# jiaowoguanren0615/Segmentation_Factory

Hardware: AMD Instinct MI355X
Metric: images/sec/GPU fwd+bwd SegFormer-B0 512x512 bf16; mIoU parity vs CPU ref (higher is better)
Workload: dtype bf16; 1 GPU; SegFormer-B0 (MiT-B0 + 768-wide SegFormerHead as the reference builds it), 150 classes, 512x512, full train step (zero_grad+fwd+CE/Dice+bwd+AGC/AdamW); per_gpu_batch=256, global_batch=256, parallelism=dp1, fp8=False, inputs=resident in HBM in the captured step's input buffers (zero-copy feed), launch=hipGraph(zero_grad+fwd+loss+bwd+grad gather) + RCCL all-reduce + fused AGC/AdamW

## Files before the change

### include/segfac.h

```cpp
#ifndef SEGFAC_H
#define SEGFAC_H
#include <stdint.h>

#ifdef __cplusplus
extern "C" {
#endif

#define SEGF_F32 0
#define SEGF_BF16 1
#define SEGF_ERR_SHAPE (-1)
#define SEGF_ERR_DTYPE (-2)
#define SEGF_ERR_WORKSPACE (-3)

const char* segf_version(void);

int segf_cast(const void* src, int src_dt, void* dst, int dst_dt, int64_t n, void* stream);
int segf_cast2d(const void* src, int src_dt, int64_t ld_src, void* dst, int dst_dt, int64_t ld_dst, int64_t rows, int64_t cols,
                void* stream);
int segf_permute021(const void* in, int in_dt, void* out, int out_dt, int64_t A, int64_t Bd, int64_t Cd,
                    int64_t ld_out, void* stream);
typedef struct SegfPrepItem {
    const void* src; void* dst;
    int64_t rows, cols, ld_src, ld_dst, pb, pc;
    int32_t op, src_dt, dst_dt, reserved;
// ... 119 lines not shown
                         float* ws, const void* x1, int64_t ldx1, int C1, float* dG, float* dwcls, void* stream);

int64_t segf_grn_ws(int B, int64_t rows_per_sample, int C, int bwd);
int segf_grn_fwd(int dt, int B, int64_t rows_per_sample, int C, const void* x, const float* gamma, const float* beta, void* y,
                 float* a_scratch, float* sumsq_out, float* ws, int pre_gelu, void* stream);
int segf_grn_bwd(int dt, int B, int64_t rows_per_sample, int C, const void* x, const void* dy, const float* gamma,
                 const float* sumsq_saved, void* dx, float* dgamma, float* dbeta, float* ws, int pre_gelu, void* stream);

int segf_attention_fwd(int dt, int B, int heads, int N, int Nkv, int hd, const void* q, int64_t ldq,
                       const void* k, int64_t ldk, const void* v, int64_t ldv, float scale,
                       void* o, int64_t ldo, float* lse, void* stream);
int64_t segf_attention_bwd_ws(int B, int heads, int N, int Nkv, int hd);
int segf_attention_bwd(int dt, int B, int heads, int N, int Nkv, int hd, const void* q, int64_t ldq,
                       const void* k, int64_t ldk, const void* v, int64_t ldv, float scale,
                       const void* o, int64_t ldo, const void* d_o, int64_t lddo, const float* lse,
                       void* dq, int64_t lddq, void* dk, int64_t lddk, void* dv, int64_t lddv,
                       float* ws, void* stream);

int segf_dwconv3x3_gelu_fwd(int dt, int B, int H, int W, int C, const void* x, const float* w ,
                            const float* bias, int apply_gelu, void* y, void* stream);
int64_t segf_dwconv3x3_bwd_ws(int B, int H, int W, int C);
int segf_dwconv3x3_bwd_blocks(int dt, int B, int H, int W, int C);
int segf_dwconv3x3_gelu_bwd(int dt, int B, int H, int W, int C, const void* x, const float* w, const float* bias,
                            int apply_gelu, const void* dy, void* du, void* dx, float* dw, float* db,
                            float* ws, void* stream);

int segf_dwconv7x7_fwd(int dt, int B, int H, int W, int C, const void* x, const float* wt, const float* bias, void* y,
                       void* stream);
int64_t segf_dwconv7x7_bwd_ws(int B, int H, int W, int C);
int segf_dwconv7x7_bwd(int dt, int B, int H, int W, int C, const void* x, const float* wt, const void* dy, void* dx,
                       float* dw, float* db, float* ws, void* stream);

int segf_conv3x3_fwd_splitk(int mode, int B, int H, int W, int Cin, int Cout);
int segf_conv3x3_pick_splitk(int Cin, int Cout, int64_t P);
int segf_conv3x3(int mode, int B, int H, int W, int Cin, int Cout, const void* x, int64_t ldx, const void* w, int64_t ldw,
                 void* y, int y_dt, int64_t ldy, const float* bias, int split_k, float* ws, void* stream);

int segf_gelu(int dt, int mode, const void* u, const void* dy, void* y, int64_t n, void* stream);
int segf_rowdot(const float* a, int64_t lda, const float* b, int64_t ldb, const float* extra_a, const float* extra_b,
                float* out, int64_t rows, int64_t cols, void* stream);
int segf_adaptive_avgpool(int dt, int bwd, int B, int H, int W, int C, int S, const void* in, void* out, void* stream);

int segf_im2col(int dt, int in_nchw_f32, int B, int H, int W, int Cin, int kh, int kw, int stride, int pad,
                int Ho, int Wo, const void* x, void* col, int64_t ldcol, void* stream);
int segf_col2im(int dt, int B, int H, int W, int Cin, int kh, int kw, int stride, int pad,
                int Ho, int Wo, const void* dcol, int64_t ldcol, void* dx, void* stream);

int segf_bilinear_fwd(int dt, int B, int h, int w, int C, const void* in, int64_t ldi,
                      int H, int W, void* out, int64_t ldo, int align_corners, void* stream);
int segf_bilinear_bwd(int dt, int B, int h, int w, int C, void* din, int64_t ldi,
                      int H, int W, const void* dout, int64_t ldo, int align_corners, void* stream);
int segf_bilinear_bwd_248(int dt, int B, int H, int W, int C, const void* dout, int64_t ldo, void* d2, void* d4, void* d8,
                          void* stream);
int segf_upsample_add(int dt, int B, int H, int W, int C, const void* base, int64_t ldb, int nsrc,
                      const void* src0, int h0, int w0, int64_t ld0, const void* src1, int h1, int w1, int64_t ld1,
                      const void* src2, int h2, int w2, int64_t ld2, void* out, int64_t ldo, int align_corners, void* stream);
int64_t segf_upsample_add_stats_ws(int B, int H, int W, int C);
int segf_upsample_add_stats(int dt, int B, int H, int W, int C, const void* base, int64_t ldb, int nsrc,
                            const void* src0, int h0, int w0, int64_t ld0, const void* src1, int h1, int w1, int64_t ld1,
                            const void* src2, int h2, int w2, int64_t ld2, void* out, int64_t ldo, int align_corners,
                            float* sums, float* ws, void* stream);
int segf_fuse_map_248_supported(int dt, int B, int H, int W, int C, int C1);
int64_t segf_fuse_map_248_ws(int B, int H, int W, int C);
int segf_fuse_map_248(int B, int H, int W, int C, int C1, const void* x1, int64_t ldx1, const void* g1, int64_t ldg,
                      const void* t2, int64_t ld2, const void* t3, int64_t ld3, const void* t4, int64_t ld4,
                      void* out, int64_t ldo, float* sums, float* ws, void* stream);
int segf_bn_stats_from_sums(const float* sums, int64_t rows, int C, float* mean, float* rstd, float* running_mean,
                            float* running_var, float momentum, float eps, void* stream);
int segf_nearest_up(int dt, int bwd, int B, int h, int w, int C, int H, int W, const void* in, const void* base, void* out,
                    void* stream);
int segf_bilinear_to_nchw_f32(int dt, int B, int h, int w, int C, const void* in, int64_t ldi,
                              int H, int W, float* out, void* stream);

int64_t segf_ce_dice_stats_floats(int B, int C);
int64_t segf_ce_dice_lse_floats(int dt, int B, int C, int h, int w, int H, int W, const void* logits, int64_t ldl);
int segf_ce_dice_fwd(int dt, int B, int C, int h, int w, int H, int W, const void* logits, int64_t ldl,
                     const int64_t* target, int64_t ignore_index, const float* class_weight, int dice,
                     float* stats, float* loss, float* pix_lse, void* stream);
int64_t segf_ce_dice_bwd_ws(int dt, int B, int C, int h, int w, int H, int W);
int segf_ce_dice_bwd(int dt, int B, int C, int h, int w, int H, int W, const void* logits, int64_t ldl,
                     const int64_t* target, int64_t ignore_index, const float* class_weight, int dice,
                     const float* stats, const float* grad_out, void* dlogits, int64_t ldd, float* ws,
                     const float* pix_lse, void* stream);

int segf_debug_wave_reduce16(const float* in, float* out, void* stream);

int segf_argmax_confmat(int dt, int B, int C, int h, int w, int H, int W, const void* logits, int64_t ldl,
                        const int64_t* target, int64_t ignore_label, int64_t* mat, int64_t* hist,
                        int32_t* flag, int64_t* pred_out , void* stream);

int segf_argmax_rows(int dt, int64_t rows, int C, const void* x, int64_t ld, int64_t* out, void* stream);

int segf_confmat_pairs(const int64_t* gt, const int64_t* pred, int64_t n, int C, int64_t ignore_label,
                       int64_t* mat, int64_t* hist, int32_t* flag, void* stream);

int segf_agc_adamw(float* param, const float* grad, float* exp_avg, float* exp_avg_sq,
                   const int64_t* unit_offset, const int32_t* unit_len, const uint8_t* unit_flags, int32_t* unit_step,
                   int nunits, float lr, float beta1, float beta2, float eps, float weight_decay, int step,
                   float clip_factor, float agc_eps, void* stream);

int64_t segf_clip_grad_ws(void);
int segf_clip_grad(float* grad, int64_t n, int mode, float value, float* ws, void* stream);

typedef struct {
    const uint8_t* img;
    const uint8_t* lbl;
// ... 28 lines not shown
```

### segmentation_factory_amd/csrc/fuse_map.hip

```cpp
#include <stdlib.h>
#include "colreduce.h"

typedef __attribute__((ext_vector_type(8))) __bf16 bf16x8;
typedef __attribute__((ext_vector_type(4))) float f32x4;
typedef __attribute__((ext_vector_type(4))) short s16x4;
typedef __attribute__((ext_vector_type(8))) short s16x8;
typedef uint32_t u32x4 __attribute__((ext_vector_type(4)));

#define FM_SLICE 128
#define FM_SROW 272
#define FM_NSRC 61
#ifndef FM_OCC
#define FM_OCC 2
#endif

struct FuseMapArgs {
    const bf16_t* x1; int64_t ldx1;
    const bf16_t* g1; int64_t ldg;
    const bf16_t *src0, *src1, *src2; int64_t ld0, ld1, ld2;
    bf16_t* out; int64_t ldo;
    float* partial;
    int B, H, W, C;
    int tiles_x, tiles_per_img; int64_t ntiles;
    FastDivU32 div_tx, div_tpi;
// ... 353 lines not shown
            SEGF_LOADS_ISSUED();
        }
        if (tx <= 1 || tx == w8 - 1) build_weights(tx);
#pragma unroll
        for (int ct = 0; ct < 2; ++ct) {
            const int cb = 16 * (2 * wave + ct);
            f32x4 acc0 = {0.f, 0.f, 0.f, 0.f}, acc1 = {0.f, 0.f, 0.f, 0.f};
#pragma unroll
            for (int s = 0; s < 8; ++s) {
                const unsigned char* tile = win + (s >> 1) * 16384;
                const int gp = g ^ phase, q = mi >> 2, pp = mi & 3;
                const int u = (cb >> 2) + pp, chunk = u >> 1, half = u & 1;
                const int kr0 = 32 * (s & 1) + 8 * gp + q, kr1 = kr0 + 4;
                const s16x4 lo = __builtin_amdgcn_ds_read_tr16_b64_v4i16(
                    (__attribute__((address_space(3))) s16x4*)(tile + kr0 * 256 + ((chunk ^ fm_swz(kr0)) << 4) + half * 8));
                const s16x4 hi = __builtin_amdgcn_ds_read_tr16_b64_v4i16(
                    (__attribute__((address_space(3))) s16x4*)(tile + kr1 * 256 + ((chunk ^ fm_swz(kr1)) << 4) + half * 8));
                const bf16x8 fa = __builtin_bit_cast(bf16x8, __builtin_shufflevector(lo, hi, 0, 1, 2, 3, 4, 5, 6, 7));
                if (s >= 1 && s <= 6) acc0 = __builtin_amdgcn_mfma_f32_16x16x32_bf16(fa, wb0[s - 1], acc0, 0, 0, 0);
                acc1 = __builtin_amdgcn_mfma_f32_16x16x32_bf16(fa, wb1[s], acc1, 0, 0, 0);
            }
            *reinterpret_cast<uint2*>(ost[0] + mi * FM_SROW + (cb + 4 * g) * 2) = make_uint2(pack2bf(acc0[0], acc0[1]), pack2bf(acc0[2], acc0[3]));
            *reinterpret_cast<uint2*>(ost[1] + mi * FM_SROW + (cb + 4 * g) * 2) = make_uint2(pack2bf(acc1[0], acc1[1]), pack2bf(acc1[2], acc1[3]));
        }
        __syncthreads();
        store_half(phase, sreg);
        {
            const int src = threadIdx.x >> 4;
            const uint4 o = *reinterpret_cast<const uint4*>(ost[0] + src * FM_SROW + 16 * ck);
            *reinterpret_cast<uint4*>(a.d2 + (((int64_t)b * h2 + 4 * ty + (src >> 2)) * w2 + 4 * tx + (src & 3)) * a.C + c0 + 8 * ck) = o;
            if (threadIdx.x < 80) {
                const uint4 o1 = *reinterpret_cast<const uint4*>(ost[1] + src * FM_SROW + 16 * ck);
                bf16_t* dst = src < 4 ? a.d4 + (((int64_t)b * h4 + 2 * ty + (src >> 1)) * w4 + 2 * tx + (src & 1)) * a.C
                                      : a.d8 + (((int64_t)b * h8 + ty) * w8 + tx) * a.C;
                *reinterpret_cast<uint4*>(dst + c0 + 8 * ck) = o1;
            }
        }
        __syncthreads();
    }
}

int fuse_map_bwd_supported(int dt, int B, int H, int W, int C) {
    return dt == SEGF_BF16 && B > 0 && H % 8 == 0 && W % 8 == 0 && H >= 8 && W >= 8 && C % FM_SLICE == 0 &&
           (int64_t)H * W < (1ll << 30) && !POL(no_bwd248_mfma);
}
int fuse_map_bwd_launch(int B, int H, int W, int C, const void* dy, int64_t ldo, void* d2, void* d4, void* d8, hipStream_t st) {
    FuseMapBwdArgs a{(const bf16_t*)dy, ldo, (bf16_t*)d2, (bf16_t*)d4, (bf16_t*)d8, B, H, W, C, C / FM_SLICE};
    const int64_t wgs = (int64_t)B * (H / 8) * a.nslice;
    if (wgs <= 0 || wgs >= (1ll << 31)) return SEGF_ERR_SHAPE;
    hipLaunchKernelGGL(fuse_map_bwd_kernel, dim3((unsigned)wgs), dim3(256), 0, st, a);
    SEGF_CHECK_LAUNCH();
    return 0;
}
```

### segmentation_factory_amd/csrc/policy.h

```cpp
#pragma once

#define SEGF_POLICY_TABLE(X)                                                                                                             \
                                                                                                   \
    X(gemm_no_big, "SEGFAC_GEMM_NO_BIG", 0, "never take the 256 x 256-tile kernel (gemm_bf16_big_kernel): everything on the 128-tile one") \
    X(gemm_no_skinny, "SEGFAC_GEMM_NO_SKINNY", 0, "no streaming products for K, N <= 128 (gemm_skinny_kernel and its relatives)")        \
    X(gemm_no_skinny_rows, "SEGFAC_GEMM_NO_SKINNY_ROWS", 0, "the [tokens x 32] -> 768 projection on gemm_skinny_kernel instead of the whole-row form") \
    X(gemm_no_skinny_k, "SEGFAC_GEMM_NO_SKINNY_K", 0, "no K-split streaming product for 32- / 64-wide outputs (gemm_skinny_k_kernel)")  \
    X(gemm_no_dw_skinny, "SEGFAC_GEMM_NO_DW_SKINNY", 0, "small-output weight gradients on the tiled split-K kernel instead of gemm_dw_skinny_kernel") \
    X(gemm_no_narrow, "SEGFAC_GEMM_NO_NARROW", 0, "256-tile kernel: full 128 x 64 wave tiles also for outputs <= 160 wide (bit-identical results)") \
    X(gemm_no_deep, "SEGFAC_GEMM_NO_DEEP", 0, "256-tile forward: one K step of operand loads in flight instead of two")                  \
    X(gemm_no_deep128, "SEGFAC_GEMM_NO_DEEP128", 0, "128-tile kernel: one K step in flight instead of two")                              \
    X(gemm_no_fastload, "SEGFAC_GEMM_NO_FASTLOAD", 0, "guarded tile loads everywhere (no workgroup-uniform guard-free full-K-step loads)") \
    X(gemm_no_tr, "SEGFAC_GEMM_NO_TR", 0, "debugging: reduction-major fragments by scalar LDS reads instead of ds_read_b64_tr_b16; disables every kernel built on the transposed read") \
    X(gemm_no_pro, "SEGFAC_GEMM_NO_PRO", 0, "segf_gemm_pro_supported answers 0: BatchNorm + ReLU + Dropout2d are applied by their own pass") \
    X(gemm_no_fused_db, "SEGFAC_GEMM_NO_FUSED_DB", 0, "bias gradient as its own column-sum launch instead of riding on the weight-gradient product") \
    X(no_grouped_dw, "SEGFAC_NO_GROUPED_DW", 0, "segf_gemm_dw_db_grouped runs its members one by one")                                   \
    X(dw_no_xcd_slabs, "SEGFAC_DW_NO_XCD_SLABS", 0, "split-K weight gradients (128-tile kernel) in hardware workgroup order instead of one K slab per XCD")                \
    X(dw_no_shared_split, "SEGFAC_DW_NO_SHARED_SPLIT", 0, "grouped weight gradients keep their per-layer slice counts (also read by the host layer)") \
    X(no_wide_reduce, "SEGFAC_NO_WIDE_REDUCE", 0, "split-K partials of large outputs summed by the 16 x 16 form instead of whole rows")   \
    X(no_reduce4, "SEGFAC_NO_REDUCE4", 0, "split-K reduce: one output per thread instead of four (bitwise the same sums)")               \
    X(gemm_f32_no_mfma, "SEGFAC_GEMM_F32_NO_MFMA", 0, "fp32 storage (exact-parity mode, evaluate): products on the vector FMA kernel instead of the f32 matrix instruction") \
    X(gemm8_linear, "SEGFAC_GEMM8_LINEAR", 1, "0: plain nn.Linear products never take the eight-phase kernel (the 256 / 128 tile kernels as in r04)") \
    X(gemm8_linear_min_tiles, "SEGFAC_GEMM8_LINEAR_MIN_TILES", 128, "fewest 256 x 256 tiles for which a K >= 2048 nn.Linear product takes the eight-phase kernel (192 for shorter K)") \
    X(gemm8_linear_min_fill, "SEGFAC_GEMM8_LINEAR_MIN_FILL", 60, "smallest share (percent) of the launched 256 x 256 tiles that must be output for an nn.Linear product with ragged last tiles to take the eight-phase kernel") \
    X(gemm8_linear_min_k, "SEGFAC_GEMM8_LINEAR_MIN_K", 256, "shortest reduction for which an nn.Linear product takes the eight-phase kernel (its 12-load prologue and drain against K / 64 tiles)") \
    X(gemm8_dw, "SEGFAC_GEMM8_DW", 1, "0: nn.Linear weight gradients never take the eight-phase kernel below 65536 tokens (the grouped 128-tile kernel as in r04)") \
    X(gemm8_dw_min_gflop, "SEGFAC_GEMM8_DW_MIN_GFLOP", 100, "smallest nn.Linear weight gradient (GFLOP; both feature counts multiples of 256, >= 256 FLOP per operand byte) that takes the eight-phase kernel + a column-sum pass instead of the grouped 128-tile kernel") \
    X(gemm8_linear_min_gflop, "SEGFAC_GEMM8_LINEAR_MIN_GFLOP", 36, "smallest nn.Linear product (GFLOP, K >= 512; 100 for shorter K) that takes the eight-phase kernel") \
                                 \
    X(no_gemm8, "SEGFAC_NO_GEMM8", 0, "no eight-phase kernel at all (gemm8_kernel): the two-phase 256-tile kernel everywhere")           \
    X(no_gemm8t, "SEGFAC_NO_GEMM8T", 0, "no eight-phase kernel for weight gradients (reduction-major operands)")                         \
    X(conv_no_fwd_split, "SEGFAC_CONV_NO_FWD_SPLIT", 0, "3 x 3 forward / data gradient with few output tiles: no split over the (channel block, tap) walk") \
    X(g8_stagger, "SEGFAC_G8_STAGGER", -1, "eight-phase kernel: 1 = wave groups one barrier apart, 0 = lockstep, -1 = staggered for bf16 and the per-device choice (segf_gemm8_option) for fp8") \
    X(no_fp8, "SEGFAC_NO_FP8", 0, "segf_gemm_fp8_supported answers 0 (block-scaled 128-tile fp8 GEMM)")                                  \
    X(no_fp8_conv, "SEGFAC_NO_FP8_CONV", 0, "segf_conv3x3_fp8*_supported answer 0")                                                      \
    X(no_fp8_wgrad, "SEGFAC_NO_FP8_WGRAD", 0, "fp8 3 x 3 convolutions keep a bf16 weight gradient")                                      \
    X(no_fp8_linear, "SEGFAC_NO_FP8_LINEAR", 0, "segf_linear_fp8_supported answers 0")                                                   \
                                                                            \
    X(attn_no_mfma, "SEGFAC_ATTN_NO_MFMA", 0, "attention on the VALU reference kernels (attention.hip) also in bf16")                    \
    X(attn_f32_no_mfma, "SEGFAC_ATTN_F32_NO_MFMA", 0, "fp32 attention forward on the vector kernel (one query per lane) instead of the f32 matrix instruction") \
    X(attn64_prescale, "SEGFAC_ATTN64_PRESCALE", 0, "head dim 64, >= 128 keys: scale log2(e) rides on the Q fragments (bf16(q c), one more rounding per q element) and -max / -lse are the score accumulators' initial values, instead of one multiply-add per score: forward + query-side backward, +8 % / +2 % per kernel, attention error x 1.2 - 2.3") \
    X(attn64_dkv_rows, "SEGFAC_ATTN64_DKV_ROWS", 128, "head dim 64, >= 128 keys, key-side backward: query rows per staged Q / dO tile and barrier (128, 64 or 32: the same arithmetic, bit for bit)") \
    X(attn_no_fused_bwd, "SEGFAC_ATTN_NO_FUSED_BWD", 0, "head dim 32, <= 256 keys: query-side + key-side backward kernels instead of the one-kernel backward") \
                                                                                \
    X(dw_no_walk, "SEGFAC_DW_NO_WALK", 0, "depthwise 3 x 3: the round-1 strip kernels instead of the vertical-walk kernels")             \
    X(dw_walk_rows, "SEGFAC_DW_WALK_ROWS", 0, "depthwise 3 x 3 walk: rows per segment (0 = chosen from the map size)")                   \
    X(dw_no_small, "SEGFAC_DW_NO_SMALL", 0, "depthwise 3 x 3 backward of small maps: three passes instead of the one-launch LDS form")   \
    X(dw_small_always, "SEGFAC_DW_SMALL_ALWAYS", 0, "... the one-launch form beyond one round of workgroups as well")                    \
                                                           \
    X(no_fuse_map, "SEGFAC_NO_FUSE_MAP", 0, "folded SegFormerHead map: streaming product + VALU upsample-add instead of fuse_map_kernel") \
    X(no_bwd248_mfma, "SEGFAC_NO_BWD248_MFMA", 0, "transposed 1/2-1/4-1/8 resizes on the VALU kernel instead of fuse_map_bwd_kernel")    \
    X(upadd_generic, "SEGFAC_UPADD_GENERIC", 0, "upsample-add: the generic per-source kernels also for the 2-4-8 pyramid")               \
    X(no_head_fused, "SEGFAC_NO_HEAD_FUSED", 0, "segf_bn_cls_bwd_supported answers 0: classifier data gradient and BatchNorm backward as separate passes") \
    X(no_head_fused_dw, "SEGFAC_NO_HEAD_FUSED_DW", 0, "the folded head's stage-1 weight gradient does not ride on pass 2 of the fused BatchNorm backward") \
                                                                                 \
    X(loss_no_band, "SEGFAC_LOSS_NO_BAND", 0, "CE / Dice forward and backward on the tile kernels instead of the band sweep")            \
    X(loss_no_band_fwd, "SEGFAC_LOSS_NO_BAND_FWD", 0, "... the forward only")                                                             \
    X(loss_band_rows, "SEGFAC_LOSS_BAND_ROWS", 0, "band sweep: rows per segment (0 = 16)")                                               \
    X(loss_no_mfma, "SEGFAC_LOSS_NO_MFMA", 0, "ratio-4 loss kernels on the VALU cells form (fp32 storage)")                              \
    X(loss_no_retry, "SEGFAC_LOSS_NO_RETRY", 0, "no exact per-pixel retry pass behind the flagged cells")                                \
    X(loss_no_lse, "SEGFAC_LOSS_NO_LSE", 0, "the backward recomputes the softmax normalisation instead of taking the forward's per-pixel log-sum") \
                                                                                                 \
    X(no_wide_finalize, "SEGFAC_NO_WIDE_FINALIZE", 0, "column-reduction finalize: one output per thread instead of four (bitwise the same sums)") \
                                                                                 \
    X(no_ln_patch, "SEGFAC_NO_LN_PATCH", 0, "[host] MiT blocks: im2col / col2im around the spatial-reduction conv instead of the patch-major LayerNorm output") \
    X(no_scaled_ln_bwd, "SEGFAC_NO_SCALED_LN_BWD", 0, "[host] DropPath backward as its own scale_rows launch instead of riding on the LayerNorm backward") \
    X(no_deferred_dw, "SEGFAC_NO_DEFERRED_DW", 0, "[host] weight gradients issued layer by layer inside the captured step (no grouped launches)") \
    X(no_deferred_finalize, "SEGFAC_NO_DEFERRED_FINALIZE", 0, "[host] LayerNorm dgamma / dbeta finalizes issued one by one")              \
    X(no_head_fused_cw, "SEGFAC_NO_HEAD_FUSED_CW", 0, "[host] the classifier's weight gradient as its own product instead of riding on pass 1 of the fused BatchNorm backward") \
    X(no_bwd248, "SEGFAC_NO_BWD248", 0, "[host] folded head backward: three segf_bilinear_bwd launches instead of the one-pass segf_bilinear_bwd_248") \
    X(no_gelu_grn, "SEGFAC_NO_GELU_GRN", 0, "[host] ConvNeXtV2 blocks: GELU as its own pass in front of the GRN kernels")                \
    X(no_weight_shadow, "SEGFAC_NO_WEIGHT_SHADOW", 0, "[host] captured step: weights cast to bf16 per use instead of one cast of the flat buffer") \
    X(no_derived_weights, "SEGFAC_NO_DERIVED_WEIGHTS", 0, "[host] captured step: derived weight layouts built in front of each layer instead of one grouped launch")

struct SegfPolicy {
#define SEGF_POLICY_FIELD(field, env, def, doc) int field;
    SEGF_POLICY_TABLE(SEGF_POLICY_FIELD)
#undef SEGF_POLICY_FIELD
    int g8_stagger_fp8;
};

const SegfPolicy& segf_policy();
#define POL(field) (segf_policy().field)

struct SegfTrace {
    int on;
    int dry;
    int n;
    const char* names[256];
    const char* where[256];
};
SegfTrace& segf_trace();
void segf_trace_note(const char* kernel_text, const char* where);
```

### segmentation_factory_amd/functional.py

```python
import contextlib

import torch
from torch.autograd import Function

from . import hip


def _rowmajor(t):
    return t if t.stride(-1) == 1 else t.contiguous()


_SHADOW = None


class shadow_scope:
    def __init__(self, table):
        self.table = table

    def __enter__(self):
        global _SHADOW
        self.prev, _SHADOW = _SHADOW, self.table
        return self

    def __exit__(self, *exc):
# ... 950 lines not shown
                     ('zero', Wp[:, Ci + 1:])]
            xs.append(x)
            Wps.append(Wp)
        hip.prep_grouped(jobs)
        jobs = []
        for i in range(4):
            Ci = xs[i].shape[1]
            Fi = wfc[:, (3 - i) * E:(4 - i) * E]
            Gp = hip.gemm(1, Fi, Wps[i], E, Ci + 8, E, out_dtype=torch.float32)
            G = torch.empty((E, Ci), dtype=dtype, device=dev)
            beta_i = torch.empty(E, dtype=torch.float32, device=dev)
            jobs += [('cast', Gp[:, :Ci], G), ('cast', Gp[:, Ci:Ci + 1], beta_i.unsqueeze(1))]
            Gps.append(Gp)
            Gs.append(G)
            betas.append(beta_i)
        hip.prep_grouped(jobs)
        for i in range(4):
            x, G, beta_i, Wp = xs[i], Gs[i], betas[i], Wps[i]
            Ci = x.shape[1]
            _, h, w = geoms[i]
            if one_pass and i == 0:
                G1, beta1 = G, beta_i
                ts.append(None)
            else:
                if one_pass and i == 1:
                    beta_i = hip.add(beta_i.unsqueeze(0), beta1.unsqueeze(0)).squeeze(0)
                ts.append(hip.gemm(0, x, G, B * h * w, E, Ci, bias=beta_i))
            saved += [x, G, Wp]
            if i == 0 and ctx.fold_slot is not None and dtype == torch.bfloat16:
                ctx.fold_slot['x1'] = x
        if one_pass:
            y, sums = hip.fuse_map_248(saved[0], G1, ts[1], ts[2], ts[3], B, H1, W1)
        else:
            y, sums = hip.upsample_add_stats(ts[0], [(ts[i], geoms[i][1], geoms[i][2]) for i in range(1, 4)], B, H1, W1, E)
        if sums is None:
            sums = torch.empty(0, device=y.device)
        ctx.mark_non_differentiable(sums)
        ctx.set_materialize_grads(False)
        ctx.save_for_backward(wfc, *saved)
        ctx.meta = (geoms, E, dtype)
        return y, sums

    @staticmethod
    def backward(ctx, dy, _dsums=None):
        geoms, E, dtype = ctx.meta
        sv = ctx.saved_tensors
        wfc = sv[0]
        B, H1, W1 = geoms[0]
        dy = _rowmajor(dy)
        dev = dy.device
        dbeta = None
        dwf = torch.empty((E, 4 * E), dtype=torch.float32, device=dev)
        dxs, dws, dbs = [], [], []
        dts = None
        if (H1 % 8 == 0 and W1 % 8 == 0 and E % 8 == 0 and not hip.policy('no_bwd248')
                and all(geoms[i][1:] == (H1 >> i, W1 >> i) for i in (1, 2, 3))):
            dts = hip.bilinear_bwd_248(dy, B, H1, W1, E)
        dGps = []
        for i in range(4):
            x, G, Wp = sv[1 + 3 * i], sv[2 + 3 * i], sv[3 + 3 * i]
            _, h, w = geoms[i]
            M, Ci = x.shape
            dt = dy if i == 0 else (dts[i - 1] if dts is not None else hip.bilinear_bwd(dy, B, h, w, E, H1, W1, align_corners=False))
            dxs.append(hip.gemm(1, dt, G, M, Ci, E) if ctx.needs_input_grad[1 + i] else None)
            pre = ctx.fold_slot.pop('dG', None) if (i == 0 and ctx.fold_slot is not None) else None
            if pre is not None and tuple(pre.shape) == (E, Ci + 8):
                dGp = pre
                dbeta = dGp[:, Ci]
            else:
                dGp = torch.empty((E, Ci + 8), dtype=torch.float32, device=dev)
                if i == 0:
                    _, dbeta = hip.gemm_dw_db(dt, x, E, Ci, M, split_k=_splitk(E, Ci, M), out=dGp[:, :Ci])
                else:
                    hip.gemm(2, dt, x, E, Ci, M, out=dGp[:, :Ci], split_k=_splitk(E, Ci, M))
            dGps.append(dGp)
        dGcs, jobs = [], []
        for i in range(4):
            Ci = sv[1 + 3 * i].shape[1]
            if dtype == torch.float32:
                dGc = dGps[i]
                jobs += [('zero', dGc[:, Ci + 1:])] + ([('cast', dbeta.unsqueeze(1), dGc[:, Ci:Ci + 1])] if dbeta.data_ptr() != dGc[:, Ci].data_ptr() else [])
            else:
                dGc = torch.empty((E, Ci + 8), dtype=dtype, device=dev)
                jobs += [('cast', dGps[i][:, :Ci], dGc[:, :Ci]), ('cast', dbeta.unsqueeze(1), dGc[:, Ci:Ci + 1]), ('zero', dGc[:, Ci + 1:])]
            dGcs.append(dGc)
        hip.prep_grouped(jobs)
        for i in range(4):
            Wp, dGc = sv[3 + 3 * i], dGcs[i]
            Ci = sv[1 + 3 * i].shape[1]
            Fi = wfc[:, (3 - i) * E:(4 - i) * E]
            hip.gemm(0, dGc, Wp, E, E, Ci + 8, out=dwf[:, (3 - i) * E:(4 - i) * E])
            dWp = hip.gemm(2, Fi, dGc, E, Ci + 8, E, out_dtype=torch.float32)
            dws.append(dWp[:, :Ci])
            dbs.append(dWp[:, Ci])
        if ctx.fold_slot is not None:
            ctx.fold_slot.clear()
        return (None, *dxs, *dws, *dbs, dwf.view(E, 4 * E, 1, 1), None)


def segformer_folded_fuse(feats, weights, biases, fuse_weight, geoms):
    slot = {}
    y, sums = SegformerFoldedFuseFn.apply(tuple(geoms), *feats, *weights, *biases, fuse_weight, slot)
    y._segf_fold = slot
    return y, (sums if sums.numel() else None)


@direct_grads(1, 2)
class DWConv7Fn(Function):

    @staticmethod
    def forward(ctx, x, weight, bias, B, H, W):
        x = x if x.is_contiguous() else x.contiguous()
        Cc = x.shape[1]
        wsrc = weight.detach().contiguous()

        def make_wt():
            t = torch.empty((49, Cc), dtype=torch.float32, device=x.device)
# ... 370 lines not shown
```

### segmentation_factory_amd/hip.py

```python
import ctypes as C
import os
import re

import torch

_HERE = os.path.dirname(os.path.abspath(__file__))
LIB_PATH = os.environ.get('SEGFAC_HIP_LIB') or os.path.join(_HERE, 'libsegfac_hip.so')
HEADER_PATH = os.path.normpath(os.path.join(_HERE, '..', 'include', 'segfac.h'))
F32, BF16 = 0, 1
ERR_SHAPE = -1
_lib = None

_i, _l, _f, _p = C.c_int, C.c_int64, C.c_float, C.c_void_p
_SCALAR = {'int': _i, 'int32_t': _i, 'int64_t': _l, 'float': _f}
_POINTEE = {'void', 'char', 'int', 'int32_t', 'int64_t', 'uint8_t', 'uint64_t', 'float'}


def _ctype(ctype, where, structs):
    t = re.sub(r'\bconst\b', ' ', ctype).replace('*', ' * ').split()
    if t and all(w == '*' for w in t[1:]):
        base, stars = t[0], len(t) - 1
        if stars == 0 and base in _SCALAR:
            return _SCALAR[base]
        if stars == 1 and base == 'char':
# ... 929 lines not shown
    out = torch.empty(((B * h * w) if bwd else (B * H * W), Cc), dtype=x.dtype, device=x.device)
    _chk(lib().segf_nearest_up(dt_of(x), int(bwd), B, h, w, Cc, H, W, _ptr(x), _ptr(base), _ptr(out), _stream()), 'segf_nearest_up')
    return out


def input_train(samples, B, H, W, mean3, std3, label_lut, out_img=None, out_lbl=None):
    _need_cuda(samples, mean3, std3, label_lut)
    assert samples.dtype == torch.uint8 and samples.numel() == B * C.sizeof(InputSample)
    assert mean3.dtype == torch.float32 and std3.dtype == torch.float32 and mean3.numel() == 3 and std3.numel() == 3
    assert label_lut is None or (label_lut.dtype == torch.int64 and label_lut.numel() == 256)
    dev = samples.device
    if out_img is None:
        out_img = torch.empty((B, 3, H, W), dtype=torch.float32, device=dev)
    if out_lbl is None:
        out_lbl = torch.empty((B, H, W), dtype=torch.int64, device=dev)
    assert out_img.is_contiguous() and out_lbl.is_contiguous() and out_img.numel() == B * 3 * H * W and out_lbl.numel() == B * H * W
    lsum = torch.empty(max(B, 2), dtype=torch.int64, device=dev)
    _chk(lib().segf_input_train(_ptr(samples), B, H, W, _ptr(lsum), _ptr(mean3), _ptr(std3), _ptr(label_lut), _ptr(out_img),
                                _ptr(out_lbl), _stream()), 'segf_input_train')
    return out_img, out_lbl


def input_val(img, lbl, out_h, out_w, mean3, std3, label_lut):
    _need_cuda(img, lbl, mean3, std3, label_lut)
    assert img.dtype == torch.uint8 and lbl.dtype == torch.uint8 and img.dim() == 3 and img.shape[2] == 3 and img.stride(2) == 1 \
        and img.stride(1) == 3 and lbl.stride(1) == 1 and lbl.shape == img.shape[:2]
    assert label_lut is None or (label_lut.dtype == torch.int64 and label_lut.numel() == 256)
    h, w = int(img.shape[0]), int(img.shape[1])
    ws = torch.empty(int(lib().segf_input_val_ws(h, w, out_h, out_w)) + 16, dtype=torch.uint8, device=img.device)
    out_img = torch.empty((3, out_h, out_w), dtype=torch.float32, device=img.device)
    out_lbl = torch.empty((out_h, out_w), dtype=torch.int64, device=img.device)
    _chk(lib().segf_input_val(_ptr(img), img.stride(0), _ptr(lbl), lbl.stride(0), h, w, out_h, out_w, _ptr(ws), _ptr(mean3),
                              _ptr(std3), _ptr(label_lut), _ptr(out_img), _ptr(out_lbl), _stream()), 'segf_input_val')
    return out_img, out_lbl


def infer_preprocess(img, out_h, out_w, mean3, std3):
    _need_cuda(img, mean3, std3)
    assert img.dtype == torch.uint8 and img.dim() == 3 and img.shape[0] == 3 and img.is_contiguous()
    out = torch.empty((1, 3, out_h, out_w), dtype=torch.float32, device=img.device)
    _chk(lib().segf_infer_preprocess(_ptr(img), int(img.shape[1]), int(img.shape[2]), out_h, out_w, _ptr(mean3), _ptr(std3), _ptr(out),
                                     _stream()), 'segf_infer_preprocess')
    return out


def bilinear_bwd_248(dout, B, H, W, Cc):
    _need_cuda(dout)
    outs = [torch.empty((B * (H // r) * (W // r), Cc), dtype=dout.dtype, device=dout.device) for r in (2, 4, 8)]
    _chk(lib().segf_bilinear_bwd_248(dt_of(dout), B, H, W, Cc, _ptr(dout), dout.stride(0), _ptr(outs[0]), _ptr(outs[1]),
                                     _ptr(outs[2]), _stream()), 'segf_bilinear_bwd_248')
    return outs


def upsample_add(base, srcs, B, H, W, Cc, align_corners=False):
    out = torch.empty((B * H * W, Cc), dtype=base.dtype, device=base.device)
    a = []
    for k in range(3):
        if k < len(srcs):
            t, h, w = srcs[k]
            a += [_ptr(t), h, w, t.stride(0)]
        else:
            a += [None, 0, 0, 0]
    _chk(lib().segf_upsample_add(dt_of(base), B, H, W, Cc, _ptr(base), base.stride(0), len(srcs), *a, _ptr(out), Cc,
                                 int(align_corners), _stream()), 'segf_upsample_add')
    return out


def upsample_add_stats(base, srcs, B, H, W, Cc):
    out = torch.empty((B * H * W, Cc), dtype=base.dtype, device=base.device)
    a = []
    for k in range(3):
        if k < len(srcs):
            t, h, w = srcs[k]
            a += [_ptr(t), h, w, t.stride(0)]
        else:
            a += [None, 0, 0, 0]
    sums = torch.empty((2, Cc), dtype=torch.float32, device=base.device)
    ws = _f32(max(1, lib().segf_upsample_add_stats_ws(B, H, W, Cc)), base.device)
    rc = lib().segf_upsample_add_stats(dt_of(base), B, H, W, Cc, _ptr(base), base.stride(0), len(srcs), *a, _ptr(out), Cc, 0,
                                       _ptr(sums), _ptr(ws), _stream())
    if rc == ERR_SHAPE:
        return upsample_add(base, srcs, B, H, W, Cc), None
    _chk(rc, 'segf_upsample_add_stats')
    return out, sums


def fuse_map_248_supported(dtype, B, H, W, Cc, C1):
    return dtype == torch.bfloat16 and bool(lib().segf_fuse_map_248_supported(BF16, B, H, W, Cc, C1))


def fuse_map_248(x1, g1, t2, t3, t4, B, H, W, with_sums=True):
    _need_cuda(x1, g1, t2, t3, t4)
    Cc, C1 = g1.shape
    out = torch.empty((B * H * W, Cc), dtype=torch.bfloat16, device=x1.device)
    sums = torch.empty((2, Cc), dtype=torch.float32, device=x1.device) if with_sums else None
    ws = _f32(max(1, lib().segf_fuse_map_248_ws(B, H, W, Cc)), x1.device) if with_sums else None
    _chk(lib().segf_fuse_map_248(B, H, W, Cc, C1, _ptr(x1), x1.stride(0), _ptr(g1), g1.stride(0), _ptr(t2), t2.stride(0),
                                 _ptr(t3), t3.stride(0), _ptr(t4), t4.stride(0), _ptr(out), Cc,
                                 _ptr(sums) if with_sums else None, _ptr(ws) if with_sums else None, _stream()), 'segf_fuse_map_248')
    return out, sums


def bn_stats_from_sums(sums, rows, running_mean, running_var, momentum, eps):
    Cc = sums.shape[1]
    mean = torch.empty(Cc, dtype=torch.float32, device=sums.device)
    rstd = torch.empty(Cc, dtype=torch.float32, device=sums.device)
# ... 65 lines not shown
```

Before: 4648 images/sec.

## Fuse stage-1 data gradient GEMM into the 2-4-8 bilinear backward kernel

Adds a kernel that, while streaming the head's map gradient through LDS to produce the 1/2, 1/4 and 1/8 transposed-resize gradients, also multiplies each resident tile by the stage-1 weights G1 to emit the stage-1 input gradient. This replaces the separate GEMM that reread the full-resolution map gradient. In exchange it adds register pressure for the per-block accumulators, extra LDS for G1 fragments, and a different work split across workgroups (runs of blocks per row instead of channel slices). It is gated on C1==32, bf16, and enough workgroups.

Result: no change. 4652 images/sec (median of 6 runs) (+0.1%).

```diff
diff --git a/include/segfac.h b/include/segfac.h
--- a/include/segfac.h
+++ b/include/segfac.h
@@ -195,6 +195,9 @@
                       int H, int W, const void* dout, int64_t ldo, int align_corners, void* stream);
 int segf_bilinear_bwd_248(int dt, int B, int H, int W, int C, const void* dout, int64_t ldo, void* d2, void* d4, void* d8,
                           void* stream);
+int segf_bilinear_bwd_248_dx1_supported(int dt, int B, int H, int W, int C, int C1);
+int segf_bilinear_bwd_248_dx1(int dt, int B, int H, int W, int C, const void* dout, int64_t ldo, void* d2, void* d4, void* d8,
+                              const void* g1, int64_t ldg, int C1, void* dx1, int64_t ldx1, void* stream);
 int segf_upsample_add(int dt, int B, int H, int W, int C, const void* base, int64_t ldb, int nsrc,
                       const void* src0, int h0, int w0, int64_t ld0, const void* src1, int h1, int w1, int64_t ld1,
                       const void* src2, int h2, int w2, int64_t ld2, void* out, int64_t ldo, int align_corners, void* stream);
diff --git a/segmentation_factory_amd/csrc/fuse_map.hip b/segmentation_factory_amd/csrc/fuse_map.hip
--- a/segmentation_factory_amd/csrc/fuse_map.hip
+++ b/segmentation_factory_amd/csrc/fuse_map.hip
@@ -429,3 +429,215 @@
     SEGF_CHECK_LAUNCH();
     return 0;
 }
+
+struct FuseMapBwdDx1Args {
+    const bf16_t* dy; int64_t ldo;
+    bf16_t *d2, *d4, *d8;
+    const bf16_t* g1; int64_t ldg;
+    bf16_t* dx1; int64_t ldx1;
+    int B, H, W, C;
+    int nslice, runs_x;
+};
+
+template <int R, int NT>
+__global__ void __launch_bounds__(256, 2) fuse_map_bwd_dx1_kernel(FuseMapBwdDx1Args a) {
+    __shared__ __attribute__((aligned(16))) unsigned char win[4 * 64 * 256];
+    __shared__ __attribute__((aligned(16))) unsigned char ost0[16 * FM_SROW];
+    __shared__ __attribute__((aligned(16))) unsigned char ost1[5 * FM_SROW];
+    __shared__ __attribute__((aligned(16))) unsigned char g1lds[4 * NT * 1024];
+    const int lane = threadIdx.x & 63, wave = threadIdx.x >> 6;
+    const int mi = lane & 15, g = lane >> 4;
+    const unsigned L = xcd_block();
+    const int rx = (int)(L % (unsigned)a.runs_x);
+    const unsigned row = L / (unsigned)a.runs_x;
+    const int h8 = a.H >> 3, w8 = a.W >> 3;
+    const int ty = (int)(row % (unsigned)h8), b = (int)(row / (unsigned)h8);
+    const int tx0 = rx * R, nblk = w8 - tx0 < R ? w8 - tx0 : R;
+    const int h2 = a.H >> 1, w2 = a.W >> 1, h4 = a.H >> 2, w4 = a.W >> 2;
+
+    const int l1 = mi < 4 ? 1 : 2, oy1 = mi < 4 ? (mi >> 1) : 0, ox1 = mi < 4 ? (mi & 1) : 0;
+    const bool live1 = mi < 5;
+    float wy0[6], wy1[8];
+#pragma unroll
+    for (int s = 0; s < 8; ++s) {
+        const int wy = 2 * s + (g >> 1);
+        if (s >= 1 && s <= 6) wy0[s - 1] = fmb_w1d(0, mi >> 2, wy, ty, h8);
+        wy1[s] = live1 ? fmb_w1d(l1, oy1, wy, ty, h8) : 0.f;
+    }
+    bf16x8 wb0[6], wb1[8];
+    auto build_weights = [&](int tx) {
+        float wx0[8], wx1[8];
+#pragma unroll
+        for (int j = 0; j < 8; ++j) {
+            const int wx = 8 * (g & 1) + j;
+            wx0[j] = fmb_w1d(0, mi & 3, wx, tx, w8);
+            wx1[j] = live1 ? fmb_w1d(l1, ox1, wx, tx, w8) : 0.f;
+        }
+#pragma unroll
+        for (int s = 0; s < 8; ++s) {
+            if (s >= 1 && s <= 6) {
+                union { uint32_t u[4]; bf16x8 v; } f;
+#pragma unroll
+                for (int j = 0; j < 4; ++j) f.u[j] = pack2bf(wy0[s - 1] * wx0[2 * j], wy0[s - 1] * wx0[2 * j + 1]);
+                wb0[s - 1] = f.v;
+            }
+            union { uint32_t u[4]; bf16x8 v; } f1;
+#pragma unroll
+            for (int j = 0; j < 4; ++j) f1.u[j] = pack2bf(wy1[s] * wx1[2 * j], wy1[s] * wx1[2 * j + 1]);
+            wb1[s] = f1.v;
+        }
+    };
+    const int ck = threadIdx.x & 15, p0 = threadIdx.x >> 4;
+    const bf16_t* imgbase = a.dy + (int64_t)b * a.H * a.W * a.ldo + 8 * ck;
+    int yoff[8];
+#pragma unroll
+    for (int i = 0; i < 8; ++i) {
+        int y = 8 * ty - 4 + ((p0 + 16 * i) >> 3);
+        y = y < 0 ? 0 : (y > a.H - 1 ? a.H - 1 : y);
+        yoff[i] = y * a.W;
+    }
+    auto load_half = [&](int c0, int col0, u32x4 (&reg)[8]) {
+        int x = col0 + (p0 & 7);
+        x = x < 0 ? 0 : (x > a.W - 1 ? a.W - 1 : x);
+#pragma unroll
+        for (int i = 0; i < 8; ++i) reg[i] = *reinterpret_cast<const u32x4*>(imgbase + (int64_t)(yoff[i] + x) * a.ldo + c0);
+    };
+    auto store_half = [&](int phys, const u32x4 (&reg)[8]) {
+#pragma unroll
+        for (int i = 0; i < 8; ++i) {
+            const int p = p0 + 16 * i, wy = p >> 3, wxh = p & 7;
+            const int krow = 32 * ((wy & 3) >> 1) + 16 * (wy & 1) + 8 * phys + wxh;
+            *reinterpret_cast<u32x4*>(win + (wy >> 2) * 16384 + krow * 256 + ((ck ^ fm_swz(krow)) << 4)) = reg[i];
+        }
+    };
+
+    const int cy = 4 + 2 * wave + (mi >> 3), cx = 4 + (mi & 7);
+    const unsigned char* ctile = win + (cy >> 2) * 16384;
+    const int crow0 = 32 * ((cy & 3) >> 1) + 16 * (cy & 1) + (cx & 7);
+    const int gn = 8 * (mi >> 2) + (mi & 3);
+    f32x4 dacc[R][NT];
+#pragma unroll
+    for (int j = 0; j < R; ++j)
+#pragma unroll
+        for (int nt = 0; nt < NT; ++nt) dacc[j][nt] = f32x4{0.f, 0.f, 0.f, 0.f};
+
+    u32x4 sreg[8];
+    load_half(0, 8 * tx0 - 4, sreg);
+    for (int slice = 0; slice < a.nslice; ++slice) {
+        const int c0 = slice * FM_SLICE;
+        store_half(0, sreg);
+        load_half(c0, 8 * tx0 + 4, sreg);
+#pragma unroll
+        for (int f = wave; f < 4 * NT; f += 4) {
+            const int nt = f >> 2, s = f & 3;
+            const bf16_t* gp = a.g1 + (int64_t)(c0 + 32 * s + 8 * g) * a.ldg + 32 * (nt >> 1) + 4 * (nt & 1) + gn;
+            s16x8 w;
+#pragma unroll
+            for (int j = 0; j < 8; ++j) w[j] = (short)gp[(int64_t)j * a.ldg];
+            *reinterpret_cast<s16x8*>(g1lds + f * 1024 + lane * 16) = w;
+        }
+        store_half(1, sreg);
+        __syncthreads();
+        for (int j = 0; j < nblk; ++j) {
+            const int tx = tx0 + j, phase = j & 1;
+            const bool last = j + 1 == nblk;
+            {
+                const int cn = !last ? c0 : (slice + 1 < a.nslice ? c0 + FM_SLICE : c0);
+                const int coln = !last ? 8 * tx + 12 : (slice + 1 < a.nslice ? 8 * tx0 - 4 : 8 * tx + 4);
+                load_half(cn, coln, sreg);
+                SEGF_LOADS_ISSUED();
+            }
+            if (j == 0 || tx <= 1 || tx == w8 - 1) build_weights(tx);
+#pragma unroll
+            for (int ct = 0; ct < 2; ++ct) {
+                const int cb = 16 * (2 * wave + ct);
+                f32x4 acc0 = {0.f, 0.f, 0.f, 0.f}, acc1 = {0.f, 0.f, 0.f, 0.f};
+#pragma unroll
+                for (int s = 0; s < 8; ++s) {
+                    const unsigned char* tile = win + (s >> 1) * 16384;
+                    const int gp = g ^ phase, q = mi >> 2, pp = mi & 3;
+                    const int u = (cb >> 2) + pp, chunk = u >> 1, half = u & 1;
+                    const int kr0 = 32 * (s & 1) + 8 * gp + q, kr1 = kr0 + 4;
+                    const s16x4 lo = __builtin_amdgcn_ds_read_tr16_b64_v4i16(
+                        (__attribute__((address_space(3))) s16x4*)(tile + kr0 * 256 + ((chunk ^ fm_swz(kr0)) << 4) + half * 8));
+                    const s16x4 hi = __builtin_amdgcn_ds_read_tr16_b64_v4i16(
+                        (__attribute__((address_space(3))) s16x4*)(tile + kr1 * 256 + ((chunk ^ fm_swz(kr1)) << 4) + half * 8));
+                    const bf16x8 fa = __builtin_bit_cast(bf16x8, __builtin_shufflevector(lo, hi, 0, 1, 2, 3, 4, 5, 6, 7));
+                    if (s >= 1 && s <= 6) acc0 = __builtin_amdgcn_mfma_f32_16x16x32_bf16(fa, wb0[s - 1], acc0, 0, 0, 0);
+                    acc1 = __builtin_amdgcn_mfma_f32_16x16x32_bf16(fa, wb1[s], acc1, 0, 0, 0);
+                }
+                *reinterpret_cast<uint2*>(ost0 + mi * FM_SROW + (cb + 4 * g) * 2) = make_uint2(pack2bf(acc0[0], acc0[1]), pack2bf(acc0[2], acc0[3]));
+                if (live1)
+                    *reinterpret_cast<uint2*>(ost1 + mi * FM_SROW + (cb + 4 * g) * 2) = make_uint2(pack2bf(acc1[0], acc1[1]), pack2bf(acc1[2], acc1[3]));
+            }
+            {
+                const int krow = crow0 + 8 * ((cx >> 3) ^ phase);
+#pragma unroll
+                for (int s = 0; s < 4; ++s) {
+                    const bf16x8 xb = __builtin_bit_cast(bf16x8, *reinterpret_cast<const uint4*>(ctile + krow * 256 + (((4 * s + g) ^ fm_swz(krow)) << 4)));
+#pragma unroll
+                    for (int nt = 0; nt < NT; ++nt) {
+                        const bf16x8 gf = __builtin_bit_cast(bf16x8, *reinterpret_cast<const uint4*>(g1lds + (4 * nt + s) * 1024 + lane * 16));
+                        dacc[0][nt] = __builtin_amdgcn_mfma_f32_16x16x32_bf16(gf, xb, dacc[0][nt], 0, 0, 0);
+                    }
+                }
+            }
+            __syncthreads();
+            if (!last) store_half(phase, sreg);
+            {
+                const int src = threadIdx.x >> 4;
+                const uint4 o = *reinterpret_cast<const uint4*>(ost0 + src * FM_SROW + 16 * ck);
+                *reinterpret_cast<uint4*>(a.d2 + (((int64_t)b * h2 + 4 * ty + (src >> 2)) * w2 + 4 * tx + (src & 3)) * a.C + c0 + 8 * ck) = o;
+                if (threadIdx.x < 80) {
+                    const uint4 o1 = *reinterpret_cast<const uint4*>(ost1 + src * FM_SROW + 16 * ck);
+                    bf16_t* dst = src < 4 ? a.d4 + (((int64_t)b * h4 + 2 * ty + (src >> 1)) * w4 + 2 * tx + (src & 1)) * a.C
+                                          : a.d8 + (((int64_t)b * h8 + ty) * w8 + tx) * a.C;
+                    *reinterpret_cast<uint4*>(dst + c0 + 8 * ck) = o1;
+                }
+            }
+            __syncthreads();
+#pragma unroll
+            for (int i = 0; i + 1 < R; ++i)
+#pragma unroll
+                for (int nt = 0; nt < NT; ++nt) { const f32x4 t = dacc[i][nt]; dacc[i][nt] = dacc[i + 1][nt]; dacc[i + 1][nt] = t; }
+        }
+        for (int j = nblk; j < R; ++j)
+#pragma unroll
+            for (int i = 0; i + 1 < R; ++i)
+#pragma unroll
+                for (int nt = 0; nt < NT; ++nt) { const f32x4 t = dacc[i][nt]; dacc[i][nt] = dacc[i + 1][nt]; dacc[i + 1][nt] = t; }
+    }
+#pragma unroll
+    for (int j = 0; j < R; ++j) {
+        if (j < nblk) {
+            bf16_t* dst = a.dx1 + (((int64_t)b * a.H + 8 * ty + 2 * wave + (mi >> 3)) * a.W + 8 * (tx0 + j) + (mi & 7)) * a.ldx1 + 8 * g;
+#pragma unroll
+            for (int q = 0; q < NT / 2; ++q) {
+                const f32x4 lo = dacc[j][2 * q], hi = dacc[j][2 * q + 1];
+                *reinterpret_cast<uint4*>(dst + 32 * q) =
+                    make_uint4(pack2bf(lo[0], lo[1]), pack2bf(lo[2], lo[3]), pack2bf(hi[0], hi[1]), pack2bf(hi[2], hi[3]));
+            }
+        }
+    }
+}
+
+#define FMB_DX1_R 4
+extern "C" int segf_bilinear_bwd_248_dx1_supported(int dt, int B, int H, int W, int C, int C1) {
+    if (!fuse_map_bwd_supported(dt, B, H, W, C) || C1 != 32 || POL(fmb_no_dx1)) return 0;
+    return (int64_t)B * (H / 8) * ((W / 8 + FMB_DX1_R - 1) / FMB_DX1_R) >= 2 * 512;
+}
+extern "C" int segf_bilinear_bwd_248_dx1(int dt, int B, int H, int W, int C, const void* dout, int64_t ldo, void* d2, void* d4, void* d8,
+                                         const void* g1, int64_t ldg, int C1, void* dx1, int64_t ldx1, void* stream) {
+    if (!segf_bilinear_bwd_248_dx1_supported(dt, B, H, W, C, C1)) return SEGF_ERR_SHAPE;
+    if (ldo < C || (ldo % 8) || ldg < C1 || ldx1 < C1 || (ldx1 % 8)) return SEGF_ERR_SHAPE;
+    if (!dout || !d2 || !d4 || !d8 || !g1 || !dx1) return SEGF_ERR_SHAPE;
+    if (((uintptr_t)dout | (uintptr_t)d2 | (uintptr_t)d4 | (uintptr_t)d8 | (uintptr_t)dx1) % 16 || (uintptr_t)g1 % 2) return SEGF_ERR_SHAPE;
+    FuseMapBwdDx1Args a{(const bf16_t*)dout, ldo, (bf16_t*)d2, (bf16_t*)d4, (bf16_t*)d8, (const bf16_t*)g1, ldg, (bf16_t*)dx1, ldx1,
+                        B, H, W, C, C / FM_SLICE, (W / 8 + FMB_DX1_R - 1) / FMB_DX1_R};
+    const int64_t wgs = (int64_t)B * (H / 8) * a.runs_x;
+    if (wgs <= 0 || wgs >= (1ll << 31)) return SEGF_ERR_SHAPE;
+    hipStream_t st = (hipStream_t)stream;
+    hipLaunchKernelGGL((fuse_map_bwd_dx1_kernel<FMB_DX1_R, 2>), dim3((unsigned)wgs), dim3(256), 0, st, a);
+    SEGF_CHECK_LAUNCH();
+    return 0;
+}
diff --git a/segmentation_factory_amd/csrc/policy.h b/segmentation_factory_amd/csrc/policy.h
--- a/segmentation_factory_amd/csrc/policy.h
+++ b/segmentation_factory_amd/csrc/policy.h
@@ -50,6 +50,7 @@
                                                            \
     X(no_fuse_map, "SEGFAC_NO_FUSE_MAP", 0, "folded SegFormerHead map: streaming product + VALU upsample-add instead of fuse_map_kernel") \
     X(no_bwd248_mfma, "SEGFAC_NO_BWD248_MFMA", 0, "transposed 1/2-1/4-1/8 resizes on the VALU kernel instead of fuse_map_bwd_kernel")    \
+    X(fmb_no_dx1, "SEGFAC_FMB_NO_DX1", 0, "segf_bilinear_bwd_248_dx1_supported answers 0: the folded head's stage-1 data gradient as its own streaming product (a second pass over the map gradient) instead of riding on fuse_map_bwd_dx1_kernel") \
     X(upadd_generic, "SEGFAC_UPADD_GENERIC", 0, "upsample-add: the generic per-source kernels also for the 2-4-8 pyramid")               \
     X(no_head_fused, "SEGFAC_NO_HEAD_FUSED", 0, "segf_bn_cls_bwd_supported answers 0: classifier data gradient and BatchNorm backward as separate passes") \
     X(no_head_fused_dw, "SEGFAC_NO_HEAD_FUSED_DW", 0, "the folded head's stage-1 weight gradient does not ride on pass 2 of the fused BatchNorm backward") \
diff --git a/segmentation_factory_amd/functional.py b/segmentation_factory_amd/functional.py
--- a/segmentation_factory_amd/functional.py
+++ b/segmentation_factory_amd/functional.py
@@ -1026,17 +1026,24 @@
         dbeta = None
         dwf = torch.empty((E, 4 * E), dtype=torch.float32, device=dev)
         dxs, dws, dbs = [], [], []
-        dts = None
+        dts, dx1 = None, None
         if (H1 % 8 == 0 and W1 % 8 == 0 and E % 8 == 0 and not hip.policy('no_bwd248')
                 and all(geoms[i][1:] == (H1 >> i, W1 >> i) for i in (1, 2, 3))):
-            dts = hip.bilinear_bwd_248(dy, B, H1, W1, E)
+            G1 = sv[2]
+            if ctx.needs_input_grad[1] and hip.bilinear_bwd_248_dx1_supported(dy.dtype, B, H1, W1, E, G1.shape[1]):
+                *dts, dx1 = hip.bilinear_bwd_248_dx1(dy, B, H1, W1, E, G1)
+            else:
+                dts = hip.bilinear_bwd_248(dy, B, H1, W1, E)
         dGps = []
         for i in range(4):
             x, G, Wp = sv[1 + 3 * i], sv[2 + 3 * i], sv[3 + 3 * i]
             _, h, w = geoms[i]
             M, Ci = x.shape
             dt = dy if i == 0 else (dts[i - 1] if dts is not None else hip.bilinear_bwd(dy, B, h, w, E, H1, W1, align_corners=False))
-            dxs.append(hip.gemm(1, dt, G, M, Ci, E) if ctx.needs_input_grad[1 + i] else None)
+            if i == 0 and dx1 is not None:
+                dxs.append(dx1)
+            else:
+                dxs.append(hip.gemm(1, dt, G, M, Ci, E) if ctx.needs_input_grad[1 + i] else None)
             pre = ctx.fold_slot.pop('dG', None) if (i == 0 and ctx.fold_slot is not None) else None
             if pre is not None and tuple(pre.shape) == (E, Ci + 8):
                 dGp = pre
diff --git a/segmentation_factory_amd/hip.py b/segmentation_factory_amd/hip.py
--- a/segmentation_factory_amd/hip.py
+++ b/segmentation_factory_amd/hip.py
@@ -1005,6 +1005,22 @@
     return outs
 
 
+def bilinear_bwd_248_dx1_supported(dtype, B, H, W, Cc, C1):
+    return dtype == torch.bfloat16 and bool(lib().segf_bilinear_bwd_248_dx1_supported(BF16, B, H, W, Cc, C1))
+
+
+def bilinear_bwd_248_dx1(dout, B, H, W, Cc, g1):
+    _need_cuda(dout, g1)
+    assert g1.dtype == torch.bfloat16 and g1.dim() == 2 and g1.shape[0] == Cc and g1.stride(1) == 1
+    C1 = g1.shape[1]
+    outs = [torch.empty((B * (H // r) * (W // r), Cc), dtype=dout.dtype, device=dout.device) for r in (2, 4, 8)]
+    dx1 = torch.empty((B * H * W, C1), dtype=dout.dtype, device=dout.device)
+    _chk(lib().segf_bilinear_bwd_248_dx1(dt_of(dout), B, H, W, Cc, _ptr(dout), dout.stride(0), _ptr(outs[0]), _ptr(outs[1]),
+                                         _ptr(outs[2]), _ptr(g1), g1.stride(0), C1, _ptr(dx1), C1, _stream()),
+         'segf_bilinear_bwd_248_dx1')
+    return (*outs, dx1)
+
+
 def upsample_add(base, srcs, B, H, W, Cc, align_corners=False):
     out = torch.empty((B * H * W, Cc), dtype=base.dtype, device=base.device)
     a = []
```
